# MCG-NKU/E2FGVI

Measured on AMD Instinct MI355X. Metric: inpainted frames/sec at 432x240 T=10, higher is better.
Workload: dtype f32; 1 GPU; BASELINE.json configs[1]: e2fgvi 432x240 T=10 l_t=10, 1 clip(s) per GPU per forward (1 in the job), random-init weights, torch.rand frames + box mask (SURVEY.md 8d); clips_per_gpu=1, precision=fp32, kernel_selection=e2fgvi_amd/tile_table.py (checked in, deterministic: ops.py), hip_graph=True, forwards_in_flight=2

## Files before the change

e2fgvi_amd/build.py:

```python
import os
import subprocess
import sys
from concurrent.futures import ThreadPoolExecutor

HERE = os.path.dirname(os.path.abspath(__file__))
CSRC = os.path.join(HERE, "csrc")
LIB = os.path.join(CSRC, "libe2fgvi_hip.so")
FLAGS = ["--offload-arch=gfx950", "-O3", "-std=c++17", "-fPIC", "-ffp-contract=fast"]
NOPK = ["-Xclang", "-target-feature", "-Xclang", "-packed-fp32-ops"]
UNITS = [("error.hip", "error.o", []), ("conv.hip", "conv.o", []), ("conv.hip", "conv_nopk.o", NOPK + ["-DE2_NOPK_VARIANT"]),
         ("conv_bf16x.hip", "conv_bf16x.o", NOPK), ("conv_wino.hip", "conv_wino.o", NOPK), ("conv_wino.hip", "conv_wino_x3.o", NOPK + ["-DE2_WINO_X3=1"]), ("conv_wino4.hip", "conv_wino4.o", NOPK), ("conv_tail.hip", "conv_tail.o", NOPK),
         ("mdcn.hip", "mdcn.o", NOPK), ("attention.hip", "attention.o", []),
         ("attention_bf16.hip", "attention_bf16.o", NOPK), ("attention_x3.hip", "attention_x3.o", NOPK), ("misc.hip", "misc.o", NOPK),
         ("video.hip", "video.o", NOPK), ("yuv.hip", "yuv.o", NOPK), ("metrics.hip", "metrics.o", NOPK),
         ("mask_track.hip", "mask_track.o", NOPK + ["-ffp-contract=off"]),
         ("defects.hip", "defects.o", NOPK)]
NOPK_OBJECTS = ("conv_nopk.o", "conv_bf16x.o", "conv_wino.o", "conv_wino4.o", "conv_wino_x3.o", "conv_tail.o", "mdcn.o", "attention_bf16.o", "attention_x3.o", "misc.o", "video.o", "yuv.o", "metrics.o", "mask_track.o", "defects.o")
OBJDUMP = "/opt/rocm/lib/llvm/bin/llvm-objdump"


def _hipcc():
    for c in (os.environ.get("HIPCC"), "/opt/rocm/bin/hipcc"):
        if c and os.path.exists(c):
            return c
    return "hipcc"


def _stale(out, deps):
    return (not os.path.exists(out)) or any(os.path.getmtime(d) > os.path.getmtime(out) for d in deps)


def build(force=False, verbose=False, nopk_all=False, lib=None, tag=None, defines=()):
    hipcc = _hipcc()
    if tag:
        nopk_all = False
    objdir = os.path.join(CSRC, ("build_" + tag) if tag else ("build_nopk" if nopk_all else "build"))
    os.makedirs(objdir, exist_ok=True)
    out = lib or (os.path.join(CSRC, "libe2fgvi_hip_%s.so" % tag) if tag else
                  os.path.join(CSRC, "libe2fgvi_hip_nopk.so") if nopk_all else LIB)
    headers = [os.path.join(CSRC, "common.h"), os.path.join(HERE, "..", "include", "e2fgvi_hip.h"), os.path.abspath(__file__)]
    jobs = []
    for src, obj, extra in UNITS:
        sp, op = os.path.join(CSRC, src), os.path.join(objdir, obj)
        if nopk_all and not any(f == "-packed-fp32-ops" for f in extra):
            extra = extra + NOPK
        if force or _stale(op, [sp] + headers):
            jobs.append([hipcc] + FLAGS + extra + list(defines) + ["-c", sp, "-o", op])

    def run(cmd):
        if verbose:
            print(" ".join(cmd), flush=True)
        subprocess.check_call(cmd)

    with ThreadPoolExecutor(max_workers=min(4, max(1, len(jobs)))) as ex:
        list(ex.map(run, jobs))
    objs = [os.path.join(objdir, obj) for _, obj, _ in UNITS]
    if force or jobs or _stale(out, objs):
        run([hipcc, "--offload-arch=gfx950", "-shared", "-fPIC", "-o", out] + objs)
    if jobs:
        verify_isa(objdir)
        if not nopk_all:
            verify_wino_waits(objdir)
            verify_exit_reuse(objdir)
            verify_no_scratch(objdir)
            verify_no_scratch(objdir, "conv_bf16x.o", "conv_halo_x3_kernel", "split-operand halo")
            verify_no_scratch(objdir, "video.o", "restore_u8_kernel", "paste-back")
            verify_no_scratch(objdir, "video.o", "overlay_stats_kernel", "overlay sums")
            verify_no_scratch(objdir, "defects.o", "defect_", "dust and dirt")
            verify_overlay_prefetch(objdir)
            verify_no_pk_u8(objdir)
            verify_no_fma64(objdir)
    return out


def build_variant(tag, *defines):
    return build(tag=tag, defines=defines)


def device_isa(obj):
    import shutil
    import tempfile
    d = tempfile.mkdtemp(prefix="e2isa")
    try:
        local = os.path.join(d, os.path.basename(obj))
        shutil.copy(obj, local)
        subprocess.run([OBJDUMP, "--offloading", os.path.basename(obj)], cwd=d, check=True, stdout=subprocess.DEVNULL,
                       stderr=subprocess.DEVNULL)
        dev = [f for f in os.listdir(d) if "gfx950" in f]
        if not dev:
            return ""
        return subprocess.run([OBJDUMP, "-d", os.path.join(d, dev[0])], check=True, capture_output=True, text=True).stdout
    finally:
        shutil.rmtree(d, ignore_errors=True)


def verify_isa(objdir=None):
    import re
    objdir = objdir or os.path.join(CSRC, "build")
    if not os.path.exists(OBJDUMP):
        return
    for obj in NOPK_OBJECTS:
        isa = device_isa(os.path.join(objdir, obj))
        bad = re.findall(r"v_pk_(?:mul|add|fma)_f32", isa)
        if bad or not isa:
            raise RuntimeError("%s: %s" % (obj, "%d packed-fp32 instructions in a unit that must have none" % len(bad) if isa
                                           else "no gfx950 code object found"))


def verify_no_fma64(objdir=None, obj="mask_track.o"):
    import re
    objdir = objdir or os.path.join(CSRC, "build")
    if not os.path.exists(OBJDUMP):
        return 0
    isa = device_isa(os.path.join(objdir, obj))
    fused = re.findall(r"v_fma(?:c|ak|mk)?_f64", isa)
    if fused or not isa:
        raise RuntimeError("%s: %s" % (obj, "%d fused fp64 multiply-adds in a unit that must round every operation" % len(fused) if isa
                                       else "no gfx950 code object found"))
# ... 324 lines not shown
```

e2fgvi_amd/csrc/conv_bf16x.hip:

```cpp
#include "common.h"

namespace {

typedef __bf16 bf16x8 __attribute__((ext_vector_type(8)));
typedef unsigned int u32x4 __attribute__((ext_vector_type(4)));
typedef __attribute__((address_space(3))) void lds_void;

struct ConvXParams {
    const void* src[E2FGVI_MAX_SRC];
    int ld[E2FGVI_MAX_SRC];
    int coff[E2FGVI_MAX_SRC];
    int cpg[E2FGVI_MAX_SRC];
    unsigned src_bytes[E2FGVI_MAX_SRC];
    int nsrc;
    int N, H, W, Ho, Wo, KH, KW, stride, pad;
    int padx;
    int osy, osx, opy, opx, oH, oW;
    int res_bcast;
    int Cout, Cout_g, Npad;
    int M;
    int tilesM, tilesN;
    int nsteps;
    unsigned wgroup_bytes;
    long long wgroup_elems;
// ... 823 lines not shown
                    for (int tm = 0; tm < TM; ++tm) acc[tm][tn] = __builtin_amdgcn_mfma_f32_32x32x16_bf16(al[tm], bh, acc[tm][tn], 0, 0, 0);
#pragma unroll
                    for (int tm = 0; tm < TM; ++tm) acc[tm][tn] = __builtin_amdgcn_mfma_f32_32x32x16_bf16(ah[tm], bl, acc[tm][tn], 0, 0, 0);
#pragma unroll
                    for (int tm = 0; tm < TM; ++tm) acc[tm][tn] = __builtin_amdgcn_mfma_f32_32x32x16_bf16(am[tm], bm, acc[tm][tn], 0, 0, 0);
#pragma unroll
                    for (int tm = 0; tm < TM; ++tm) acc[tm][tn] = __builtin_amdgcn_mfma_f32_32x32x16_bf16(am[tm], bh, acc[tm][tn], 0, 0, 0);
#pragma unroll
                    for (int tm = 0; tm < TM; ++tm) acc[tm][tn] = __builtin_amdgcn_mfma_f32_32x32x16_bf16(ah[tm], bm, acc[tm][tn], 0, 0, 0);
#pragma unroll
                    for (int tm = 0; tm < TM; ++tm) acc[tm][tn] = __builtin_amdgcn_mfma_f32_32x32x16_bf16(ah[tm], bh, acc[tm][tn], 0, 0, 0);
                }
                __builtin_amdgcn_sched_barrier(0);
#pragma unroll
                for (int pl = 0; pl < 3; ++pl) {
#pragma unroll
                    for (int tn = 0; tn < TN; ++tn) { bq[tn][pl] = bn[tn][pl]; bn[tn][pl] = bn2[tn][pl]; }
#pragma unroll
                    for (int tm = 0; tm < TM; ++tm) aq[tm][pl] = an[tm][pl];
                }
            }
        }
        if (blk + 1 < nblk) {
            __syncthreads();
            store_patch();
            __syncthreads();
        }
    }

    const float* res = reinterpret_cast<const float*>(p.res);
    float* dst = reinterpret_cast<float*>(p.dst);
#pragma unroll
    for (int tn = 0; tn < TN; ++tn) {
        const int co = wn * 32 + i;
        if (co >= p.Cout_g) continue;
        const float bv = p.bias ? p.bias[co] : 0.f;
#pragma unroll
        for (int tm = 0; tm < TM; ++tm) {
#pragma unroll
            for (int r = 0; r < 16; ++r) {
                const int row = (r & 3) + 8 * (r >> 2) + 4 * h;
                const int oy = y0 + 2 * (wm * TM + tm) + (row >> 4), ox = x0 + (row & 15);
                if (oy >= p.Ho || ox >= p.Wo) continue;
                const long long m = ((long long)img * p.Ho + oy) * p.Wo + ox;
                float v = acc[tm][tn][r] + bv;
                if (res) v += res[m * p.res_ld + p.res_coff + co];
                v = apply_act(v, p.act, p.slope);
                dst[m * p.dst_ld + p.dst_coff + co] = v;
            }
        }
    }
}

struct PackX {
    int Cout, groups, KH, KW, nsrc;
    int cpg[E2FGVI_MAX_SRC];
    int Cout_g, Npad, Cin_g, steps_per_tap;
    int kc, ch;
    int tp_cq;
    long long total, wgroup_elems;
};

bool geometry_x(int Cout, int groups, int KH, int KW, int nsrc, const int32_t* cpg, PackX* q, bool f32 = false) {
    q->kc = f32 ? 32 : 64;
    q->ch = f32 ? 4 : 8;
    q->tp_cq = 0;
    if (Cout <= 0 || groups <= 0 || Cout % groups || KH <= 0 || KW <= 0 || nsrc < 1 || nsrc > E2FGVI_MAX_SRC) return false;
    q->Cout = Cout; q->groups = groups; q->KH = KH; q->KW = KW; q->nsrc = nsrc;
    q->Cout_g = Cout / groups;
    q->Npad = round_up(q->Cout_g, 32);
    q->Cin_g = 0;
    q->steps_per_tap = 0;
    for (int s = 0; s < E2FGVI_MAX_SRC; ++s) q->cpg[s] = 0;
    for (int s = 0; s < nsrc; ++s) {
        if (cpg[s] <= 0 || cpg[s] % q->ch) return false;
        q->cpg[s] = cpg[s];
        q->Cin_g += cpg[s];
        q->steps_per_tap += cdiv(cpg[s], q->kc);
    }
    q->wgroup_elems = (long long)KH * KW * q->steps_per_tap * q->kc * q->Npad;
    q->total = q->wgroup_elems * groups;
    return true;
}

__device__ __forceinline__ float pack_value(const float* __restrict__ w, const PackX& p, int g, int step, int koct, int n, int e) {
    if (p.tp_cq) {
        const int L = 8 * step + koct;
        const int tapk = L / p.tp_cq;
        const int chk = (L - tapk * p.tp_cq) * p.ch + e;
        if (tapk < p.KH * p.KW && chk < p.cpg[0] && n < p.Cout_g)
            return w[((long long)n * p.Cin_g + chk) * (p.KH * p.KW) + tapk];
        return 0.f;
    }
    const int tap = step / p.steps_per_tap;
    int blk = step - tap * p.steps_per_tap;
    int s = 0, prefix = 0;
    while (blk >= (p.cpg[s] + p.kc - 1) / p.kc) { blk -= (p.cpg[s] + p.kc - 1) / p.kc; prefix += p.cpg[s]; ++s; }
    const int c = blk * p.kc + koct * p.ch + e;
    if (c < p.cpg[s] && n < p.Cout_g)
        return w[((long long)(g * p.Cout_g + n) * p.Cin_g + prefix + c) * (p.KH * p.KW) + tap];
    return 0.f;
}

template <typename T>
__global__ void pack_conv_weight_x_kernel(const float* __restrict__ w, T* __restrict__ wp, const PackX p) {
    const long long idx = (long long)blockIdx.x * blockDim.x + threadIdx.x;
// ... 37 lines not shown
int launch_x(ConvXParams& p, int groups, hipStream_t st, int mode = 0) {
    p.tilesM = cdiv(p.M, BM);
    p.tilesN = cdiv(p.Cout_g, BN);
    if constexpr (PP) {
        if (mode != 2 || p.tp_cq) {
            e2fgvi_set_error("conv2d_x: the ping-pong tiles (107, 108) are for the split-operand mode without tap-packed weights");
            return E2FGVI_EUNSUP;
        }
        hipLaunchKernelGGL((conv_bf16x_kernel<BM, BN, WGM, WGN, false, 2, true>), dim3(p.tilesM * p.tilesN, groups, 1), dim3(64 * WGM * WGN), 0, st, p);
        E2_LAUNCH_CHECK("conv2d_x");
        return 0;
    } else {
    if (S3 && !(p.KH == 3 && p.KW == 3 && p.stride == 1 && p.pad == 1)) {
        e2fgvi_set_error("conv2d_x: the row-shift tiles (11..17) are for 3x3 stride-1 pad-1 layers");
        return E2FGVI_EINVAL;
    }
    if (mode == 1 || mode == 2) {
        if constexpr (!S3) {
            if (mode == 2)
                hipLaunchKernelGGL((conv_bf16x_kernel<BM, BN, WGM, WGN, false, 2>), dim3(p.tilesM * p.tilesN, groups, 1), dim3(64 * WGM * WGN), 0, st, p);
            else
                hipLaunchKernelGGL((conv_bf16x_kernel<BM, BN, WGM, WGN, false, 1>), dim3(p.tilesM * p.tilesN, groups, 1), dim3(64 * WGM * WGN), 0, st, p);
        } else {
            e2fgvi_set_error("conv2d_x: the row-shift tiles (11..18) take bf16 operands only");
            return E2FGVI_EUNSUP;
        }
    } else if (mode == 3) {
        hipLaunchKernelGGL((conv_bf16x_kernel<BM, BN, WGM, WGN, S3, 3>), dim3(p.tilesM * p.tilesN, groups, 1), dim3(64 * WGM * WGN), 0, st, p);
    } else {
        hipLaunchKernelGGL((conv_bf16x_kernel<BM, BN, WGM, WGN, S3, 0>), dim3(p.tilesM * p.tilesN, groups, 1), dim3(64 * WGM * WGN), 0, st, p);
    }
    E2_LAUNCH_CHECK("conv2d_x");
    return 0;
    }
}

template <int TH, int WGM>
int launch_halo_x3(ConvXParams& p, const e2fgvi_convx_desc* d, hipStream_t st, int mode) {
    const bool ok = mode == 2 && !d->tap_packed && d->KH == 7 && d->KW == 7 && d->stride == 1 && d->pad == 3 && d->groups == 1 &&
                    d->nsrc == 1 && d->src_cpg[0] % 16 == 0 && d->Cout <= 64 && !d->out_grid && !d->res_bcast && !d->dst_nchw &&
                    !d->dst2 && d->dst_dtype == E2FGVI_F32 && (!d->residual || d->res_dtype == E2FGVI_F32) &&
                    d->act != E2FGVI_ACT_DCNPOST;
    if (!ok) {
        e2fgvi_set_error("conv2d_x: the halo tiles (51, 52) take split-operand 7x7 stride-1 pad-3 layers: one fp32 source of a multiple "
                         "of 16 channels, no groups, at most 64 output channels, plain packing, fp32 NHWC result and residual");
        return E2FGVI_EUNSUP;
    }
    p.tilesM = p.N * cdiv(p.Ho, TH) * cdiv(p.Wo, 16);
    p.tilesN = 1;
    if (p.Cout_g <= 32)
        hipLaunchKernelGGL((conv_halo_x3_kernel<7, TH, 32, WGM>), dim3(p.tilesM, 1, 1), dim3(64 * WGM), 0, st, p);
    else
        hipLaunchKernelGGL((conv_halo_x3_kernel<7, TH, 64, WGM>), dim3(p.tilesM, 1, 1), dim3(128 * WGM), 0, st, p);
    E2_LAUNCH_CHECK("conv2d_x");
    return 0;
}

}

static bool geometry_taps(int Cout, int KH, int KW, int cin, PackX* q, bool f32 = false) {
    const int32_t cpg[1] = {cin};
    if (cin > 56 || KW < 2 || !geometry_x(Cout, 1, KH, KW, 1, cpg, q, f32)) return false;
    q->tp_cq = cin / q->ch;
    const int steps = cdiv(KH * KW * q->tp_cq, 8);
    q->wgroup_elems = (long long)steps * q->kc * q->Npad;
    q->total = q->wgroup_elems;
    return true;
}

static int mode_x(const char* who, int32_t code) {
    switch (code) {
        case E2FGVI_BF16: return 0;
        case E2FGVI_F32: return 1;
        case E2FGVI_BF16X3: return 2;
        case E2FGVI_F16: return 3;
        default: break;
    }
    e2fgvi_set_error("%s: mode %d is none of E2FGVI_F32 (0), E2FGVI_BF16 (1), E2FGVI_BF16X3 (2), E2FGVI_F16 (3)", who, code);
    return -1;
}

static bool pack_geometry(const char* who, int mode, int tap_packed, int Cout, int groups, int KH, int KW, int nsrc,
                          const int32_t* src_cpg, PackX* q) {
    const bool f32 = mode == 1 || mode == 2;
    const int ch = f32 ? 4 : 8;
    if (!src_cpg) {
        e2fgvi_set_error("%s: null src_cpg", who);
        return false;
    }
    if (tap_packed) {
        if (groups == 1 && nsrc == 1 && geometry_taps(Cout, KH, KW, src_cpg[0], q, f32)) return true;
        e2fgvi_set_error("%s: tap-packed weights: one source of %d ... 56 channels (multiple of %d), no groups, KW >= 2", who, ch, ch);
        return false;
    }
    if (geometry_x(Cout, groups, KH, KW, nsrc, src_cpg, q, f32)) return true;
    e2fgvi_set_error("%s: bad geometry (channels per source must be multiples of %d)", who, ch);
    return false;
}

extern "C" int64_t e2fgvi_packed_conv_weight_x_size(int32_t mode, int32_t tap_packed, int32_t Cout, int32_t groups, int32_t KH,
                                                    int32_t KW, int32_t nsrc, const int32_t* src_cpg) {
    PackX q;
    const int m = mode_x("packed_conv_weight_x_size", mode);
    if (m < 0 || !pack_geometry("packed_conv_weight_x_size", m, tap_packed, Cout, groups, KH, KW, nsrc, src_cpg, &q)) return E2FGVI_EINVAL;
    return m == 2 ? 3 * q.total : q.total;
}
// ... 89 lines not shown
    p.padx = d->out_grid ? d->pad_left : d->pad;
    p.osy = d->out_grid ? d->out_sy : 0; p.osx = d->out_sx; p.opy = d->out_py; p.opx = d->out_px; p.oH = d->out_H; p.oW = d->out_W;
    p.res_bcast = d->res_bcast;
    p.Cout = d->Cout; p.Cout_g = q.Cout_g; p.Npad = q.Npad;
    p.M = d->N * d->Ho * d->Wo;
    p.nsteps = d->KH * d->KW * q.steps_per_tap;
    p.tp_cq = 0; p.tp_magic = 0; p.tp_magic_cq = 0;
    if (d->tap_packed) {
        PackX qt;
        E2_REQUIRE(d->nsrc == 1 && d->groups == 1 && geometry_taps(d->Cout, d->KH, d->KW, d->src_cpg[0], &qt, f32), E2FGVI_EINVAL,
                   "conv2d_x: tap-packed weights are for one source of <= 56 channels, no groups, KW >= 2");
        E2_REQUIRE(d->tile < 10 || d->tile > 20, E2FGVI_EUNSUP, "conv2d_x: the row-shift tiles do not take tap-packed weights");
        q.wgroup_elems = qt.wgroup_elems;
        p.tp_cq = qt.tp_cq;
        p.tp_magic = 0xFFFFFFFFu / (unsigned)d->KW + 1u;
        p.tp_magic_cq = qt.tp_cq > 1 ? 0xFFFFFFFFu / (unsigned)qt.tp_cq + 1u : 0u;
        p.nsteps = cdiv(d->KH * d->KW * qt.tp_cq, 8);
    }
    p.wgroup_elems = q.wgroup_elems; p.wgroup_bytes = (unsigned)(q.wgroup_elems * wbytes_num);
    p.w = d->wpacked; p.bias = d->bias;
    p.res = d->residual; p.res_ld = d->res_ld; p.res_coff = d->res_coff; p.res_bf16 = d->res_dtype == dt16;
    p.dst = d->dst; p.dst_ld = d->dst_ld; p.dst_coff = d->dst_coff; p.dst_bf16 = d->dst_dtype == dt16;
    p.dst_nchw = d->dst_nchw;
    p.dst2 = (__bf16*)d->dst2; p.dst2_ld = d->dst2_ld; p.dst2_coff = d->dst2_coff;
    p.split_from = d->dst2_split_from; p.split_plane = d->dst2_plane_stride;
    p.act = d->act; p.slope = d->slope;
    hipStream_t st = (hipStream_t)stream;
    int tile = d->tile;
    p.dbg_noload = 0;
    if (tile == 21 || tile == 24 || tile == 26 || tile == 27) { p.dbg_noload = 1; tile -= 20; }
    if (tile == 31 || tile == 34 || tile == 36) { p.dbg_noload = 2; tile -= 30; }
    if (tile == 41 || tile == 44 || tile == 46) { p.dbg_noload = 3; tile -= 40; }
    if (tile == 61 || tile == 66) { p.dbg_noload = 8; tile -= 60; }
    if (tile == 71 || tile == 74 || tile == 76 || tile == 77) { p.dbg_noload = 16; tile -= 70; }
    if (tile == 81 || tile == 84 || tile == 86 || tile == 87) { p.dbg_noload = 32; tile -= 80; }
    if (!tile) {
        if (p.Cout_g <= 32) tile = 3;
        else if (p.Cout_g <= 64) tile = 2;
        else tile = ((long long)cdiv(p.M, 128) * cdiv(p.Cout_g, 128) * d->groups >= 384) ? 1 : 4;
    }
    switch (tile) {
        case 1: return launch_x<128, 128, 2, 2, false>(p, d->groups, st, mode);
        case 2: return launch_x<128, 64, 2, 2, false>(p, d->groups, st, mode);
        case 3: return launch_x<128, 32, 4, 1, false>(p, d->groups, st, mode);
        case 4: return launch_x<64, 128, 2, 2, false>(p, d->groups, st, mode);
        case 5: return launch_x<64, 64, 2, 2, false>(p, d->groups, st, mode);
        case 6: return launch_x<256, 128, 4, 2, false>(p, d->groups, st, mode);
        case 7: return launch_x<256, 256, 4, 2, false>(p, d->groups, st, mode);
        case 8: return launch_x<256, 192, 4, 2, false>(p, d->groups, st, mode);
        case 107: return launch_x<256, 256, 4, 2, false, true>(p, d->groups, st, mode);
        case 108: return launch_x<256, 192, 4, 2, false, true>(p, d->groups, st, mode);
        case 51: return launch_halo_x3<16, 4>(p, d, st, mode);
        case 52: return launch_halo_x3<8, 2>(p, d, st, mode);
        case 11: return launch_x<128, 128, 2, 2, true>(p, d->groups, st, mode);
        case 12: return launch_x<128, 64, 2, 2, true>(p, d->groups, st, mode);
        case 13: return launch_x<128, 32, 4, 1, true>(p, d->groups, st, mode);
        case 14: return launch_x<64, 128, 2, 2, true>(p, d->groups, st, mode);
        case 16: return launch_x<256, 128, 4, 2, true>(p, d->groups, st, mode);
        case 17: return launch_x<256, 256, 4, 2, true>(p, d->groups, st, mode);
        case 18: return launch_x<256, 64, 4, 2, true>(p, d->groups, st, mode);
        default: break;
    }
    e2fgvi_set_error("conv2d_x: unknown tile %d", tile);
    return E2FGVI_EINVAL;
}

extern "C" int e2fgvi_conv2d_x(const e2fgvi_convx_desc* d, int32_t mode, void* stream) {
    const int m = mode_x("conv2d_x", mode);
    return m < 0 ? E2FGVI_EINVAL : conv2d_x(d, stream, m);
}
```

e2fgvi_amd/ops.py:

```python
import collections
import ctypes as C
import math
import numbers
import os

import torch

from . import lib as _L

ACT_NONE, ACT_RELU, ACT_LRELU, ACT_TANH, ACT_DCNPOST = _L.ACT_NONE, _L.ACT_RELU, _L.ACT_LRELU, _L.ACT_TANH, _L.ACT_DCNPOST


def _stream():
    return C.c_void_p(torch.cuda.current_stream().cuda_stream)


def _chk(t, name, dtype=torch.float32):
    if not isinstance(t, torch.Tensor) or not t.is_cuda:
        raise TypeError("%s must be a CUDA (ROCm) tensor -- the HIP path has no CPU fallback" % name)
    if t.dtype != dtype:
        raise TypeError("%s must be %s, got %s" % (name, dtype, t.dtype))
    if not t.is_contiguous():
        raise ValueError("%s must be contiguous" % name)
    return t


def _ptr(t):
    return C.c_void_p(t.data_ptr()) if t is not None else C.c_void_p(0)


def empty_nhwc(n, h, w, c, device):
    return torch.empty((n, h, w, c), dtype=torch.float32, device=device)


TUNE_CANDIDATES = (0, 213, 223, 211, 219, 216)
WINO_CANDIDATES = (64, 132, 164, 32)
W4_CODES = {2464: (2, 64)}
_W4_MINPIX = 20000
XTUNE_CANDIDATES = (1, 4, 6, 7, 8, 2, 5, 3, 107, 108, 51, 52)
XTUNE_HALO = (51, 52)
XTUNE_ROWSHIFT = (11, 16, 17, 12, 13, 18)
X3_ENABLED = os.environ.get("E2FGVI_X3", "1") != "0"
X3_MARGIN = 0.97
X3_BASE = 30000
W3_BASE = 40000
W3_CANDIDATES = (132, 164, 32, 5132, 6064)
W3_WIDE = 6064
W3_WIDE_FALLBACK = 164
DMA_BASE = 2000


def _decode(code):
    if code >= W3_BASE:
        return "w3", code - W3_BASE
    if code >= X3_BASE:
        return "x3", code - X3_BASE
    if code in W4_CODES:
        return "w4", code
    if DMA_BASE <= code < DMA_BASE + 100:
        return "dma", code - DMA_BASE
    return "own", code


_TUNED = {}
AUTOTUNE = os.environ.get("E2FGVI_AUTOTUNE", "0") == "1"
TUNE_REPS = max(1, int(os.environ.get("E2FGVI_TUNE_REPS", "1") or 1))
TABLE_FORMAT = 2
_SIZE_FIELD = 8


def _default_tune_file():
    try:
        st = os.stat(_L.LIB_PATH)
        d = os.environ.get("E2FGVI_CACHE_DIR") or os.path.join(os.path.dirname(os.path.abspath(__file__)), ".tile_cache")
        os.makedirs(d, exist_ok=True)
        dev = "gpu"
        if torch.cuda.is_available():
            dev = "".join(ch for ch in torch.cuda.get_device_properties(0).gcnArchName.split(":")[0] if ch.isalnum())
        return os.path.join(d, "tiles_v%d_%s_%x_%x.txt" % (TABLE_FORMAT, dev, st.st_size, int(st.st_mtime)))
    except (OSError, RuntimeError):
        return None


_TUNE_FILE = None
if AUTOTUNE:
    _TUNE_FILE = os.environ.get("E2FGVI_TUNE_FILE")
    if _TUNE_FILE is None:
        _TUNE_FILE = _default_tune_file()
    elif _TUNE_FILE in ("", "0"):
        _TUNE_FILE = None
    if _TUNE_FILE and os.path.exists(_TUNE_FILE):
        import ast
        for _line in open(_TUNE_FILE):
# ... 600 lines not shown
                     out2=None if out2 is None else out2[n0:n1], tile=tile, **kw)
            return out
        kw.update(out=out, residual=residual, out2=out2)
        d = self._desc(srcs, **kw)
        if planes is not None:
            self._set_planes(d, planes, split_from, N * Ho * Wo)
        if tile == 0 and self.tune and N * Ho * Wo >= 2048:
            family, tile = self._select(d, srcs, kw)
            if family == "x3":
                try:
                    return self.alt3(srcs, out_dtype=out_dtype, tile=tile, planes=planes, split_from=split_from, **kw)
                except _L.HipError:
                    tile = 0
        d.tile = tile
        if _L.TRACE is not None:
            _L.annotate(**self._work(d))
        d.wpacked = self.wpacked.data_ptr()
        rc = self._fn(C.byref(d), _stream())
        if rc != 0 and d.tile and self.tune:
            d.tile = 0
            rc = self._fn(C.byref(d), _stream())
        _L.check(rc, "conv2d_x")
        return out

    def _select(self, d, srcs, kw):
        out, residual = kw["out"], kw["residual"]
        x3 = self.try_x3 and X3_ENABLED and self.f32 and not self.x3
        key = (("x3" if self.x3 else ("x32+3" if x3 else "x32")) if self.f32 else "x", self.Cout, tuple(self.cpg), self.KH, self.KW, self.stride, self.pad, self.groups,
               int(4.0 * math.log2(d.N * d.Ho * d.Wo)), _dt_key(out), kw["out_nchw"], self.taps)
        best = _decision(key)
        if best is None and AUTOTUNE and not torch.cuda.is_current_stream_capturing() and (
                residual is None or residual.data_ptr() != out.data_ptr()):
            best = _remember(key, self._tune(d, srcs, kw, x3))
        if _decode(best or 0)[0] in ("x3", "w3"):
            return ("x3", best - X3_BASE) if self._alt3() is not None else ("own", 0)
        return "own", best or 0

    def _tune(self, d, srcs, kw, x3):
        res = self._time_tiles(d)
        best = min(res, key=res.get) if res else 0
        if x3 and self._alt3() is not None:
            res3 = self.alt3._time_tiles(self.alt3._desc(srcs, **kw))
            if res3 and (not res or min(res3.values()) < X3_MARGIN * min(res.values())):
                best = X3_BASE + min(res3, key=res3.get)
        return best

    def _work(self, d):
        N, H, W, Ho, Wo, tile = d.N, d.H, d.W, d.Ho, d.Wo, d.tile
        cin_g, cout_g, K2 = sum(self.cpg), self.Cout // self.groups, self.KH * self.KW
        kc = 32 if self.f32 else 64
        cin_p = sum(-(-c // kc) * kc for c in self.cpg)
        if self.taps:
            cin_p = -(-K2 * (self.cpg[0] // (4 if self.f32 else 8)) // 8) * kc / K2
        return dict(layer=self.name, kernel="conv_%s tile=%d%s" % (("f32x3" if self.x3 else "f32x") if self.f32 else
                                                                   "f16x" if self.f16 else "bf16x", tile, " taps" if self.taps else ""),
                    shape="N%d %dx%d %d->%d k%d s%d g%d" % (N, H, W, cin_g * self.groups, self.Cout, self.KH, self.stride, self.groups),
                    macs=N * Ho * Wo * self.Cout * cin_g * K2, tile=int(tile),
                    issued=int(N * Ho * Wo * (-(-cout_g // 32) * 32) * self.groups * cin_p * K2 * (_L.X3_PIPE if self.x3 else 1)))

    def _halo_x3(self):
        return (self.x3 and not self.taps and (self.KH, self.KW, self.stride, self.pad, self.groups) == (7, 7, 1, 3, 1)
                and len(self.cpg) == 1 and self.cpg[0] % 16 == 0 and self.Cout <= 64)

    def _time_tiles(self, d, reps=3, rounds=2):
        st = _stream()
        res = {}
        d.tile = 0
        d.wpacked = self.wpacked.data_ptr()

        def run():
            return self._fn(C.byref(d), st)
        for _ in range(2):
            run()
        for _ in range(rounds * TUNE_REPS):
            rowshift = (self.KH, self.KW, self.stride, self.pad) == (3, 3, 1, 1) and not self.f32 and not self.taps
            for code in XTUNE_CANDIDATES + (XTUNE_ROWSHIFT if rowshift else ()):
                if code in XTUNE_HALO and not self._halo_x3():
                    continue
                if code % 10 == 3 and self.Cout // self.groups > 64:
                    continue
                if code in (12, 18) and self.Cout // self.groups > 64:
                    continue
                d.tile = code
                if run() == 0:
                    res[code] = min(res.get(code, float("inf")), _time_launches(run, reps))
        d.tile = 0
        return res


class SoftCompGather:

    def __init__(self, weight, bias, channels=128, dtype=torch.bfloat16):
        w = _chk(weight.detach().float().contiguous(), "weight")
        if w.dim() != 2 or w.shape[0] != 49 * channels:
            raise ValueError("SoftComp embedding weight must be [%d, hidden]" % (49 * channels))
        self.C, self.hidden, self.dtype = channels, w.shape[1], dtype
        w4 = w.view(channels, 7, 7, self.hidden)
        self.phases = []
        for py in range(3):
            ky_taps = [6, 3, 0] if py == 0 else [py + 3, py]
            for px in range(3):
                kx_taps = [6, 3, 0] if px == 0 else [px + 3, px]
                wp = w4[:, ky_taps][:, :, kx_taps].permute(0, 3, 1, 2).contiguous()
                layer = PackedConvX(wp, None, [self.hidden], dtype=dtype)
                layer.name = "sc.embedding phase (%d,%d)" % (py, px)
                self.phases.append((py, px, 1 if py == 0 else 0, 1 if px == 0 else 0, layer))
        self.bias = None if bias is None else _chk(bias.detach().float().contiguous(), "bias")
        self._bias_img = {}
        self.tile = 0

    def bias_image(self, fh, fw):
        if self.bias is None:
            return None

        def build():
            rows = self.bias.view(self.C, 49).t().reshape(1, 49 * self.C).expand(fh * fw, 49 * self.C).contiguous()
            return softcomp_fold(rows, 1, fh, fw, 3 * fh, 3 * fw, self.C)[0].contiguous()
        return _lazy(self._bias_img, (fh, fw), "sc.embedding (folded bias image)", build)

    def __call__(self, tokens, out=None, out_dtype=None):
        _chk(tokens, "tokens", self.dtype)
        F_, fh, fw, hid = tokens.shape
        if hid != self.hidden:
            raise ValueError("tokens must be [F, fh, fw, %d]" % self.hidden)
        H, W = 3 * fh, 3 * fw
        if out is None:
            out = torch.empty((F_, H, W, self.C), dtype=out_dtype or self.dtype, device=tokens.device)
        if tuple(out.shape) != (F_, H, W, self.C):
            raise ValueError("out must be [%d,%d,%d,%d]" % (F_, H, W, self.C))
        chunks = list(_image_chunks(F_, fh * fw * hid * tokens.element_size()))
# ... 1036 lines not shown
```

e2fgvi_amd/tile_table.py:

```python
TABLE_FORMAT = 2
TILES = {
    ('x', 128, (128, 128), 1, 1, 1, 0, 1, 63, 1, False, False): 1,
    ('x', 128, (128, 128), 1, 1, 1, 0, 1, 76, 1, False, False): 4,
    ('x', 128, (128, 128), 1, 1, 1, 0, 1, 85, 1, False, False): 4,
    ('x', 128, (128, 128), 3, 3, 1, 1, 1, 50, 1, False, False): 5,
    ('x', 128, (128, 128), 3, 3, 1, 1, 1, 63, 1, False, False): 1,
    ('x', 128, (128, 128), 3, 3, 1, 1, 1, 68, 1, False, False): 4,
    ('x', 128, (128, 128, 128), 3, 3, 1, 1, 1, 50, 1, False, False): 5,
    ('x', 128, (128, 128, 128), 3, 3, 1, 1, 1, 63, 1, False, False): 11,
    ('x', 128, (128, 128, 128), 3, 3, 1, 1, 1, 68, 1, False, False): 4,
    ('x', 128, (128, 128, 128, 8), 3, 3, 1, 1, 1, 50, 1, False, False): 5,
    ('x', 128, (128, 128, 128, 8), 3, 3, 1, 1, 1, 63, 1, False, False): 11,
    ('x', 128, (128, 128, 128, 8), 3, 3, 1, 1, 1, 68, 1, False, False): 11,
    ('x', 128, (128,), 3, 3, 1, 1, 1, 50, 1, False, False): 5,
    ('x', 128, (128,), 3, 3, 1, 1, 1, 63, 1, False, False): 6,
    ('x', 128, (128,), 3, 3, 1, 1, 1, 68, 1, False, False): 4,
    ('x', 128, (128,), 3, 3, 1, 1, 1, 71, 1, False, False): 1,
    ('x', 128, (128,), 3, 3, 1, 1, 1, 76, 1, False, False): 1,
    ('x', 128, (128,), 3, 3, 1, 1, 1, 84, 1, False, False): 1,
    ('x', 128, (128,), 3, 3, 1, 1, 1, 85, 1, False, False): 6,
    ('x', 128, (128,), 3, 3, 1, 1, 1, 93, 1, False, False): 6,
    ('x', 128, (256, 256), 3, 3, 1, 1, 1, 63, 1, False, False): 16,
    ('x', 128, (256, 256), 3, 3, 1, 1, 1, 76, 1, False, False): 11,
    ('x', 128, (256, 256), 3, 3, 1, 1, 1, 85, 1, False, False): 11,
# ... 255 lines not shown
    (32, (64,), 7, 7, 1, 3, 1, 32, 49, False, 1, False, False, 0, 'x3'): 0,
    (32, (64,), 7, 7, 1, 3, 1, 32, 52, False, 1, False, False, 0, 'x3'): 0,
    (32, (64,), 7, 7, 1, 3, 1, 32, 53, False, 1, False, False, 0, 'x3'): 0,
    (32, (64,), 7, 7, 1, 3, 1, 32, 56, False, 1, False, False, 0, 'x3'): 0,
    (32, (64,), 7, 7, 1, 3, 1, 32, 57, False, 1, False, False, 0, 'x3'): 0,
    (32, (64,), 7, 7, 1, 3, 1, 32, 60, False, 1, False, False, 0, 'x3'): 30051,
    (32, (64,), 7, 7, 1, 3, 1, 32, 61, False, 1, False, False, 0, 'x3'): 30003,
    (32, (64,), 7, 7, 1, 3, 1, 32, 64, False, 1, False, False, 0, 'x3'): 30003,
    (32, (64,), 7, 7, 1, 3, 1, 32, 65, False, 1, False, False, 0, 'x3'): 30003,
    (32, (64,), 7, 7, 1, 3, 1, 32, 68, False, 1, False, False, 0, 'x3'): 30051,
    (32, (64,), 7, 7, 1, 3, 1, 32, 69, False, 1, False, False, 0, 'x3'): 30003,
    (32, (64,), 7, 7, 1, 3, 1, 32, 72, False, 1, False, False, 0, 'x3'): 30003,
    (32, (64,), 7, 7, 1, 3, 1, 32, 73, False, 1, False, False, 0, 'x3'): 30003,
    (32, (64,), 7, 7, 1, 3, 1, 32, 80, False, 1, False, False, 0, 'x3'): 30003,
    (32, (8,), 7, 7, 1, 3, 1, 8, 44, False, 1, False, False, 0, 'x3'): 0,
    (32, (8,), 7, 7, 1, 3, 1, 8, 45, False, 1, False, False, 0, 'x3'): 0,
    (32, (8,), 7, 7, 1, 3, 1, 8, 48, False, 1, False, False, 0, 'x3'): 0,
    (32, (8,), 7, 7, 1, 3, 1, 8, 49, False, 1, False, False, 0, 'x3'): 0,
    (32, (8,), 7, 7, 1, 3, 1, 8, 52, False, 1, False, False, 0, 'x3'): 0,
    (32, (8,), 7, 7, 1, 3, 1, 8, 53, False, 1, False, False, 0, 'x3'): 0,
    (32, (8,), 7, 7, 1, 3, 1, 8, 56, False, 1, False, False, 0, 'x3'): 0,
    (32, (8,), 7, 7, 1, 3, 1, 8, 57, False, 1, False, False, 0, 'x3'): 0,
    (32, (8,), 7, 7, 1, 3, 1, 8, 60, False, 1, False, False, 0, 'x3'): 0,
    (32, (8,), 7, 7, 1, 3, 1, 8, 61, False, 1, False, False, 0, 'x3'): 0,
    (32, (8,), 7, 7, 1, 3, 1, 8, 64, False, 1, False, False, 0, 'x3'): 0,
    (32, (8,), 7, 7, 1, 3, 1, 8, 65, False, 1, False, False, 0, 'x3'): 0,
    (32, (8,), 7, 7, 1, 3, 1, 8, 68, False, 1, False, False, 0, 'x3'): 0,
    (32, (8,), 7, 7, 1, 3, 1, 8, 69, False, 1, False, False, 0, 'x3'): 0,
    (32, (8,), 7, 7, 1, 3, 1, 8, 72, False, 1, False, False, 0, 'x3'): 0,
    (32, (8,), 7, 7, 1, 3, 1, 8, 73, False, 1, False, False, 0, 'x3'): 0,
    (32, (8,), 7, 7, 1, 3, 1, 8, 80, False, 1, False, False, 0, 'x3'): 0,
    (384, (256,), 3, 3, 1, 1, 1, 32, 59, False, 2, True, False, 2464, 'x3'): 46064,
    (384, (256,), 3, 3, 1, 1, 1, 32, 63, False, 2, True, False, 2464, 'x3'): 46064,
    (384, (256,), 3, 3, 1, 1, 1, 32, 67, False, 2, True, False, 2464, 'x3'): 46064,
    (384, (256,), 3, 3, 1, 1, 1, 32, 68, False, 2, True, False, 0, 'x3'): 46064,
    (384, (256,), 3, 3, 1, 1, 1, 32, 75, False, 2, True, False, 2464, 'x3'): 46064,
    (384, (64, 128), 3, 3, 1, 1, 4, 32, 59, False, 2, True, False, 0, 'x3'): 45132,
    (384, (64, 128), 3, 3, 1, 1, 4, 32, 63, False, 2, True, False, 0, 'x3'): 45132,
    (384, (64, 128), 3, 3, 1, 1, 4, 32, 67, False, 2, True, False, 0, 'x3'): 45132,
    (384, (64, 128), 3, 3, 1, 1, 4, 32, 68, False, 2, True, False, 0, 'x3'): 46064,
    (384, (64, 128), 3, 3, 1, 1, 4, 32, 75, False, 2, True, False, 0, 'x3'): 46064,
    (432, (128,), 3, 3, 1, 1, 1, 32, 50, True, 4, True, False, 0, 'x3'): 46064,
    (432, (128,), 3, 3, 1, 1, 1, 32, 54, True, 4, True, False, 0, 'x3'): 46064,
    (432, (128,), 3, 3, 1, 1, 1, 32, 55, True, 4, True, False, 0, 'x3'): 46064,
    (432, (128,), 3, 3, 1, 1, 1, 32, 62, True, 4, True, False, 0, 'x3'): 46064,
    (512, (128, 192), 3, 3, 1, 1, 2, 32, 59, False, 2, True, False, 2464, 'x3'): 46064,
    (512, (128, 192), 3, 3, 1, 1, 2, 32, 63, False, 2, True, False, 2464, 'x3'): 46064,
    (512, (128, 192), 3, 3, 1, 1, 2, 32, 67, False, 2, True, False, 2464, 'x3'): 46064,
    (512, (128, 192), 3, 3, 1, 1, 2, 32, 68, False, 2, True, False, 0, 'x3'): 46064,
    (512, (128, 192), 3, 3, 1, 1, 2, 32, 75, False, 2, True, False, 2464, 'x3'): 46064,
    (512, (128,), 7, 7, 3, 3, 1, 32, 47, False, 0, False, True, 0): 2005,
    (512, (128,), 7, 7, 3, 3, 1, 32, 47, False, 0, False, True, 0, 'x3'): 30005,
    (512, (128,), 7, 7, 3, 3, 1, 32, 51, False, 0, False, True, 0): 2004,
    (512, (128,), 7, 7, 3, 3, 1, 32, 51, False, 0, False, True, 0, 'x3'): 30004,
    (512, (128,), 7, 7, 3, 3, 1, 32, 54, False, 0, False, True, 0): 2005,
    (512, (128,), 7, 7, 3, 3, 1, 32, 54, False, 0, False, True, 0, 'x3'): 30006,
    (512, (128,), 7, 7, 3, 3, 1, 32, 55, False, 0, False, True, 0): 2001,
    (512, (128,), 7, 7, 3, 3, 1, 32, 55, False, 0, False, True, 0, 'x3'): 30001,
    (512, (128,), 7, 7, 3, 3, 1, 32, 63, False, 0, False, True, 0): 2004,
    (512, (128,), 7, 7, 3, 3, 1, 32, 63, False, 0, False, True, 0, 'x3'): 30107,
    (512, (1960,), 1, 1, 1, 0, 1, 32, 47, True, 0, False, True, 0): 2005,
    (512, (1960,), 1, 1, 1, 0, 1, 32, 51, True, 0, False, True, 0): 2004,
    (512, (1960,), 1, 1, 1, 0, 1, 32, 54, True, 0, False, True, 0): 2005,
    (512, (1960,), 1, 1, 1, 0, 1, 32, 55, True, 0, False, True, 0): 2001,
    (512, (1960,), 1, 1, 1, 0, 1, 32, 63, True, 0, False, True, 0): 2004,
    (512, (512,), 1, 1, 1, 0, 1, 32, 47, True, 0, False, True, 0): 2005,
    (512, (512,), 1, 1, 1, 0, 1, 32, 47, True, 0, False, True, 0, 'x3'): 30005,
    (512, (512,), 1, 1, 1, 0, 1, 32, 51, True, 0, False, True, 0): 2004,
    (512, (512,), 1, 1, 1, 0, 1, 32, 51, True, 0, False, True, 0, 'x3'): 30004,
    (512, (512,), 1, 1, 1, 0, 1, 32, 54, True, 0, False, True, 0): 2005,
    (512, (512,), 1, 1, 1, 0, 1, 32, 54, True, 0, False, True, 0, 'x3'): 30001,
    (512, (512,), 1, 1, 1, 0, 1, 32, 55, True, 0, False, True, 0): 2001,
    (512, (512,), 1, 1, 1, 0, 1, 32, 55, True, 0, False, True, 0, 'x3'): 30001,
    (512, (512,), 1, 1, 1, 0, 1, 32, 63, True, 0, False, True, 0): 2005,
    (512, (512,), 1, 1, 1, 0, 1, 32, 63, True, 0, False, True, 0, 'x3'): 30107,
    (6272, (512,), 1, 1, 1, 0, 1, 32, 47, False, 0, False, True, 0): 2004,
    (6272, (512,), 1, 1, 1, 0, 1, 32, 47, False, 0, False, True, 0, 'x3'): 30108,
    (6272, (512,), 1, 1, 1, 0, 1, 32, 51, False, 0, False, True, 0): 2004,
    (6272, (512,), 1, 1, 1, 0, 1, 32, 51, False, 0, False, True, 0, 'x3'): 30107,
    (6272, (512,), 1, 1, 1, 0, 1, 32, 54, False, 0, False, True, 0): 2007,
    (6272, (512,), 1, 1, 1, 0, 1, 32, 54, False, 0, False, True, 0, 'x3'): 30107,
    (6272, (512,), 1, 1, 1, 0, 1, 32, 55, False, 0, False, True, 0): 2002,
    (6272, (512,), 1, 1, 1, 0, 1, 32, 55, False, 0, False, True, 0, 'x3'): 30107,
    (6272, (512,), 1, 1, 1, 0, 1, 32, 63, False, 0, False, True, 0): 2007,
    (6272, (512,), 1, 1, 1, 0, 1, 32, 63, False, 0, False, True, 0, 'x3'): 30107,
    (64, (128,), 3, 3, 1, 1, 1, 32, 67, False, 2, True, False, 0, 'x3'): 46064,
    (64, (128,), 3, 3, 1, 1, 1, 32, 71, False, 2, True, False, 0, 'x3'): 46064,
    (64, (128,), 3, 3, 1, 1, 1, 32, 75, False, 2, True, False, 0, 'x3'): 46064,
    (64, (128,), 3, 3, 1, 1, 1, 32, 76, False, 2, True, False, 0, 'x3'): 46064,
    (64, (128,), 3, 3, 1, 1, 1, 32, 83, False, 2, True, False, 0, 'x3'): 46064,
    (64, (32,), 7, 7, 1, 3, 1, 32, 44, False, 1, False, False, 0, 'x3'): 0,
    (64, (32,), 7, 7, 1, 3, 1, 32, 45, False, 1, False, False, 0, 'x3'): 0,
    (64, (32,), 7, 7, 1, 3, 1, 32, 48, False, 1, False, False, 0, 'x3'): 0,
    (64, (32,), 7, 7, 1, 3, 1, 32, 49, False, 1, False, False, 0, 'x3'): 0,
    (64, (32,), 7, 7, 1, 3, 1, 32, 52, False, 1, False, False, 0, 'x3'): 30052,
    (64, (32,), 7, 7, 1, 3, 1, 32, 53, False, 1, False, False, 0, 'x3'): 0,
    (64, (32,), 7, 7, 1, 3, 1, 32, 56, False, 1, False, False, 0, 'x3'): 0,
    (64, (32,), 7, 7, 1, 3, 1, 32, 57, False, 1, False, False, 0, 'x3'): 30005,
    (64, (32,), 7, 7, 1, 3, 1, 32, 60, False, 1, False, False, 0, 'x3'): 30051,
    (64, (32,), 7, 7, 1, 3, 1, 32, 61, False, 1, False, False, 0, 'x3'): 30005,
    (64, (32,), 7, 7, 1, 3, 1, 32, 64, False, 1, False, False, 0, 'x3'): 30002,
    (64, (32,), 7, 7, 1, 3, 1, 32, 65, False, 1, False, False, 0, 'x3'): 30005,
    (64, (32,), 7, 7, 1, 3, 1, 32, 68, False, 1, False, False, 0, 'x3'): 30052,
    (64, (32,), 7, 7, 1, 3, 1, 32, 69, False, 1, False, False, 0, 'x3'): 30005,
    (64, (32,), 7, 7, 1, 3, 1, 32, 72, False, 1, False, False, 0, 'x3'): 30005,
    (64, (32,), 7, 7, 1, 3, 1, 32, 73, False, 1, False, False, 0, 'x3'): 30005,
    (64, (32,), 7, 7, 1, 3, 1, 32, 80, False, 1, False, False, 0, 'x3'): 30005,
# ... 15 lines not shown
```

Measured before the change: 964.2 frames/s.

## Add halo-tiled split-bf16 kernel for 7x7 stride-3 convolution

Adds a dedicated split-operand (3x bf16) MFMA kernel for 7x7 stride-3 pad-3 convolutions. Each workgroup stages an input halo patch in LDS, de-interleaved by column phase, and reuses it across all 49 taps while weights stream through a register pipeline. This targets the redundant global/im2col traffic of the generic path. The tile table switches one 512-channel stride-3 layer at 51 rows to the new tile, and the autotuner and cost model learn the new codes. Output tiles of 5x6 use 30 of 32 MFMA rows, wasting some compute.

```diff
diff --git a/e2fgvi_amd/build.py b/e2fgvi_amd/build.py
--- a/e2fgvi_amd/build.py
+++ b/e2fgvi_amd/build.py
@@ -64,6 +64,7 @@
             verify_exit_reuse(objdir)
             verify_no_scratch(objdir)
             verify_no_scratch(objdir, "conv_bf16x.o", "conv_halo_x3_kernel", "split-operand halo")
+            verify_no_scratch(objdir, "conv_bf16x.o", "conv_halo_s3_x3_kernel", "split-operand stride-3 halo")
             verify_no_scratch(objdir, "video.o", "restore_u8_kernel", "paste-back")
             verify_no_scratch(objdir, "video.o", "overlay_stats_kernel", "overlay sums")
             verify_no_scratch(objdir, "defects.o", "defect_", "dust and dirt")
diff --git a/e2fgvi_amd/csrc/conv_bf16x.hip b/e2fgvi_amd/csrc/conv_bf16x.hip
--- a/e2fgvi_amd/csrc/conv_bf16x.hip
+++ b/e2fgvi_amd/csrc/conv_bf16x.hip
@@ -899,6 +899,216 @@
     }
 }
 
+template <int TMY, int TMX, int BN, int TN>
+__global__ __launch_bounds__(64 * (BN / (32 * TN))) __attribute__((amdgpu_waves_per_eu(2))) void conv_halo_s3_x3_kernel(const ConvXParams p) {
+    constexpr int TM = TMY * TMX;
+    constexpr int TH = 5 * TMY, TW = 6 * TMX;
+    constexpr int PH = 3 * (TH - 1) + 7, PW = 3 * (TW - 1) + 7, NPIX = PH * PW;
+    constexpr int PWC = TW + 2;
+    constexpr int RP = (3 * PWC + 13) / 16 * 16 + 2;
+    constexpr int PLANE = PH * RP * 16;
+    constexpr int WGN = BN / (32 * TN);
+    constexpr int NT = 64 * WGN;
+    constexpr int P_IT = (NPIX + NT - 1) / NT;
+    constexpr int NJ = 25;
+    constexpr int BD = 2;
+    constexpr unsigned OOB = 0xFFFFFFFFu;
+    constexpr int NP = TM / 2;
+    static_assert(RP >= 3 * PWC && RP % 16 == 2 && 3 * PLANE <= 160 * 1024 && 2 * PLANE + 7 * RP * 16 < 65536, "patch");
+    static_assert(TM == 2 * NP && (NP == 1 || NP == 2), "sub-tile pairs");
+
+    __shared__ __attribute__((aligned(16))) unsigned char smem[3 * PLANE];
+
+    const int tid = threadIdx.x;
+    const int lane = tid & 63, wn = tid >> 6;
+    const int tiles_x = (p.Wo + TW - 1) / TW, tiles_y = (p.Ho + TH - 1) / TH;
+    int sp = xcd_remap(blockIdx.x, p.tilesM * p.tilesN);
+    const int n0 = (sp / p.tilesM) * BN;
+    sp %= p.tilesM;
+    const int txi = sp % tiles_x;
+    sp /= tiles_x;
+    const int tyi = sp % tiles_y;
+    const int img = sp / tiles_y;
+    const int y0 = tyi * TH, x0 = txi * TW;
+
+    int pp_pix[P_IT], pp_lds[P_IT];
+#pragma unroll
+    for (int it = 0; it < P_IT; ++it) {
+        const int f = tid + it * NT;
+        const int py = f / PW, px = f - py * PW;
+        const int iy = 3 * y0 - 3 + py, ix = 3 * x0 - 3 + px;
+        const bool ok = f < NPIX && iy >= 0 && iy < p.H && ix >= 0 && ix < p.W;
+        pp_pix[it] = ok ? (img * p.H + iy) * p.W + ix : -1;
+        pp_lds[it] = (py * RP + (px % 3) * PWC + px / 3) * 16;
+    }
+    const __amdgpu_buffer_rsrc_t arsrc = make_rsrc(p.src[0], p.src_bytes[0]);
+    const unsigned ld4 = (unsigned)p.ld[0] * 4u;
+    const unsigned chan = (unsigned)p.coff[0] * 4u;
+    const int nblk = p.cpg[0] >> 3;
+
+    f32x4 rp[P_IT][2];
+    auto load_patch = [&](int blk) {
+#pragma unroll
+        for (int it = 0; it < P_IT; ++it) {
+            const bool ok = blk < nblk && pp_pix[it] >= 0;
+            const unsigned off = (unsigned)pp_pix[it] * ld4 + chan + (unsigned)blk * 32u;
+            rp[it][0] = __builtin_bit_cast(f32x4, __builtin_amdgcn_raw_buffer_load_b128(arsrc, (int)(ok ? off : OOB), 0, 0));
+            rp[it][1] = __builtin_bit_cast(f32x4, __builtin_amdgcn_raw_buffer_load_b128(arsrc, (int)(ok ? off + 16u : OOB), 0, 0));
+        }
+    };
+    auto store_patch = [&]() {
+#pragma unroll
+        for (int it = 0; it < P_IT; ++it) {
+            if (NPIX % NT == 0 || (tid + it * NT) < NPIX) {
+                bf16x8 sh, sm, sl;
+                split8(rp[it][0], rp[it][1], sh, sm, sl);
+                *reinterpret_cast<bf16x8*>(smem + pp_lds[it]) = sh;
+                *reinterpret_cast<bf16x8*>(smem + PLANE + pp_lds[it]) = sm;
+                *reinterpret_cast<bf16x8*>(smem + 2 * PLANE + pp_lds[it]) = sl;
+            }
+        }
+    };
+
+    const int i = lane & 31;
+    const int h = lane >> 5;
+    int hm = -h;
+    const int lty = i < 30 ? i / 6 : 0, ltx = i < 30 ? i - lty * 6 : i - 16;
+    int a_base[TM];
+#pragma unroll
+    for (int tm = 0; tm < TM; ++tm) a_base[tm] = (3 * (5 * (tm / TMX) + lty) * RP + 6 * (tm % TMX) + ltx) * 16;
+    auto load_a = [&](bf16x8 (&a)[2][3], int pr, int j) {
+        const int t0 = 2 * j, t1 = 2 * j + 1 < 49 ? 2 * j + 1 : 48;
+        const int o0 = ((t0 / 7) * RP + ((t0 % 7) % 3) * PWC + (t0 % 7) / 3) * 16;
+        const int o1 = ((t1 / 7) * RP + ((t1 % 7) % 3) * PWC + (t1 % 7) / 3) * 16;
+        const int o = hm & (o1 - o0);
+#pragma unroll
+        for (int tm = 0; tm < 2; ++tm)
+#pragma unroll
+            for (int pl = 0; pl < 3; ++pl) a[tm][pl] = *reinterpret_cast<const bf16x8*>(smem + pl * PLANE + o0 + a_base[2 * pr + tm] + o);
+    };
+
+    const __amdgpu_buffer_rsrc_t wrsrc = make_rsrc(p.w, p.wgroup_bytes);
+    unsigned b_col[TN];
+#pragma unroll
+    for (int tn = 0; tn < TN; ++tn) {
+        const int col = n0 + (wn * TN + tn) * 32 + i;
+        b_col[tn] = col < p.Npad ? (unsigned)col * 16u : OOB;
+    }
+    const unsigned oct_bytes = (unsigned)p.Npad * 16u;
+    const unsigned plane_bytes = 4u * oct_bytes, step_bytes = 3u * plane_bytes;
+    const int opt = p.tp_cq ? p.tp_cq >> 1 : ((p.cpg[0] + 31) >> 5) * 4;
+    auto load_b = [&](bf16x8 (&b)[TN][3], int j, int blk) {
+        const int oc0 = 2 * j * opt + blk, oc1 = oc0 + opt;
+        const unsigned s0 = (unsigned)(oc0 >> 2) * step_bytes + (unsigned)(oc0 & 3) * oct_bytes;
+        const unsigned s1 = (unsigned)(oc1 >> 2) * step_bytes + (unsigned)(oc1 & 3) * oct_bytes;
+        const bool live0 = blk < nblk, live1 = live0 && 2 * j + 1 < 49;
+        const unsigned so = h ? s1 : s0;
+        const bool live = h ? live1 : live0;
+#pragma unroll
+        for (int tn = 0; tn < TN; ++tn) {
+            const unsigned voff = (live && b_col[tn] != OOB) ? b_col[tn] + so : OOB;
+#pragma unroll
+            for (int pl = 0; pl < 3; ++pl)
+                b[tn][pl] = __builtin_bit_cast(bf16x8, __builtin_amdgcn_raw_buffer_load_b128(wrsrc, (int)voff, (int)((unsigned)pl * plane_bytes), 0));
+        }
+    };
+
+    f32x16 acc[TM][TN];
+#pragma unroll
+    for (int tm = 0; tm < TM; ++tm)
+#pragma unroll
+        for (int tn = 0; tn < TN; ++tn)
+#pragma unroll
+            for (int r = 0; r < 16; ++r) acc[tm][tn][r] = 0.f;
+
+    bf16x8 bs[BD + 1][TN][3], aq[NP][2][3], an[2][3];
+    load_patch(0);
+#pragma unroll
+    for (int k = 0; k < BD; ++k) load_b(bs[k], k, 0);
+    store_patch();
+    __syncthreads();
+
+    auto mma_pair = [&](const bf16x8 (&a)[2][3], int pr) {
+#pragma unroll
+        for (int tn = 0; tn < TN; ++tn) {
+            const bf16x8 bh = bs[0][tn][0], bm = bs[0][tn][1], bl = bs[0][tn][2];
+#pragma unroll
+            for (int tm = 0; tm < 2; ++tm) acc[2 * pr + tm][tn] = __builtin_amdgcn_mfma_f32_32x32x16_bf16(a[tm][2], bh, acc[2 * pr + tm][tn], 0, 0, 0);
+#pragma unroll
+            for (int tm = 0; tm < 2; ++tm) acc[2 * pr + tm][tn] = __builtin_amdgcn_mfma_f32_32x32x16_bf16(a[tm][0], bl, acc[2 * pr + tm][tn], 0, 0, 0);
+#pragma unroll
+            for (int tm = 0; tm < 2; ++tm) acc[2 * pr + tm][tn] = __builtin_amdgcn_mfma_f32_32x32x16_bf16(a[tm][1], bm, acc[2 * pr + tm][tn], 0, 0, 0);
+#pragma unroll
+            for (int tm = 0; tm < 2; ++tm) acc[2 * pr + tm][tn] = __builtin_amdgcn_mfma_f32_32x32x16_bf16(a[tm][1], bh, acc[2 * pr + tm][tn], 0, 0, 0);
+#pragma unroll
+            for (int tm = 0; tm < 2; ++tm) acc[2 * pr + tm][tn] = __builtin_amdgcn_mfma_f32_32x32x16_bf16(a[tm][0], bm, acc[2 * pr + tm][tn], 0, 0, 0);
+#pragma unroll
+            for (int tm = 0; tm < 2; ++tm) acc[2 * pr + tm][tn] = __builtin_amdgcn_mfma_f32_32x32x16_bf16(a[tm][0], bh, acc[2 * pr + tm][tn], 0, 0, 0);
+        }
+    };
+
+    for (int blk = 0; blk < nblk; ++blk) {
+        asm volatile("" : "+v"(hm));
+        load_patch(blk + 1);
+        load_a(aq[0], 0, 0);
+#pragma unroll
+        for (int j = 0; j < NJ; ++j) {
+            load_b(bs[BD], j + BD < NJ ? j + BD : j + BD - NJ, j + BD < NJ ? blk : blk + 1);
+            if (NP == 2) load_a(aq[NP - 1], 1, j);
+            else if (j + 1 < NJ) load_a(an, 0, j + 1);
+            __builtin_amdgcn_sched_barrier(0);
+            mma_pair(aq[0], 0);
+            __builtin_amdgcn_sched_barrier(0);
+            if (NP == 2) {
+                if (j + 1 < NJ) load_a(an, 0, j + 1);
+                __builtin_amdgcn_sched_barrier(0);
+                mma_pair(aq[NP - 1], 1);
+                __builtin_amdgcn_sched_barrier(0);
+            }
+#pragma unroll
+            for (int pl = 0; pl < 3; ++pl) {
+#pragma unroll
+                for (int tn = 0; tn < TN; ++tn)
+#pragma unroll
+                    for (int k = 0; k < BD; ++k) bs[k][tn][pl] = bs[k + 1][tn][pl];
+                if (j + 1 < NJ) {
+#pragma unroll
+                    for (int tm = 0; tm < 2; ++tm) aq[0][tm][pl] = an[tm][pl];
+                }
+            }
+        }
+        if (blk + 1 < nblk) {
+            __syncthreads();
+            store_patch();
+            __syncthreads();
+        }
+    }
+
+    const float* res = reinterpret_cast<const float*>(p.res);
+    float* dst = reinterpret_cast<float*>(p.dst);
+#pragma unroll
+    for (int tn = 0; tn < TN; ++tn) {
+        const int co = n0 + (wn * TN + tn) * 32 + i;
+        if (co >= p.Cout_g) continue;
+        const float bv = p.bias ? p.bias[co] : 0.f;
+#pragma unroll
+        for (int tm = 0; tm < TM; ++tm) {
+#pragma unroll
+            for (int r = 0; r < 16; ++r) {
+                const int row = (r & 3) + 8 * (r >> 2) + 4 * h;
+                const int ty = row / 6;
+                const int oy = y0 + 5 * (tm / TMX) + ty, ox = x0 + 6 * (tm % TMX) + row - 6 * ty;
+                if (row >= 30 || oy >= p.Ho || ox >= p.Wo) continue;
+                const long long m = ((long long)img * p.Ho + oy) * p.Wo + ox;
+                float v = acc[tm][tn][r] + bv;
+                if (res) v += res[m * p.res_ld + p.res_coff + co];
+                v = apply_act(v, p.act, p.slope);
+                dst[m * p.dst_ld + p.dst_coff + co] = v;
+            }
+        }
+    }
+}
+
 struct PackX {
     int Cout, groups, KH, KW, nsrc;
     int cpg[E2FGVI_MAX_SRC];
@@ -1042,6 +1252,23 @@
         hipLaunchKernelGGL((conv_halo_x3_kernel<7, TH, 32, WGM>), dim3(p.tilesM, 1, 1), dim3(64 * WGM), 0, st, p);
     else
         hipLaunchKernelGGL((conv_halo_x3_kernel<7, TH, 64, WGM>), dim3(p.tilesM, 1, 1), dim3(128 * WGM), 0, st, p);
+    E2_LAUNCH_CHECK("conv2d_x");
+    return 0;
+}
+
+template <int TMY, int BN, int TN>
+int launch_halo_s3_x3(ConvXParams& p, const e2fgvi_convx_desc* d, hipStream_t st, int mode) {
+    const bool ok = mode == 2 && d->KH == 7 && d->KW == 7 && d->stride == 3 && d->pad == 3 && d->groups == 1 && d->nsrc == 1 &&
+                    d->src_cpg[0] % 8 == 0 && !d->out_grid && !d->res_bcast && !d->dst_nchw && !d->dst2 &&
+                    d->dst_dtype == E2FGVI_F32 && (!d->residual || d->res_dtype == E2FGVI_F32) && d->act != E2FGVI_ACT_DCNPOST;
+    if (!ok) {
+        e2fgvi_set_error("conv2d_x: the stride-3 halo tiles (54, 56) take split-operand 7x7 stride-3 pad-3 layers: one fp32 source of a "
+                         "multiple of 8 channels, no groups, fp32 NHWC result and residual, no second output");
+        return E2FGVI_EUNSUP;
+    }
+    p.tilesM = p.N * cdiv(p.Ho, 5 * TMY) * cdiv(p.Wo, 12);
+    p.tilesN = cdiv(p.Cout_g, BN);
+    hipLaunchKernelGGL((conv_halo_s3_x3_kernel<TMY, 2, BN, TN>), dim3(p.tilesM * p.tilesN, 1, 1), dim3(64 * (BN / (32 * TN))), 0, st, p);
     E2_LAUNCH_CHECK("conv2d_x");
     return 0;
 }
@@ -1237,6 +1464,8 @@
         case 108: return launch_x<256, 192, 4, 2, false, true>(p, d->groups, st, mode);
         case 51: return launch_halo_x3<16, 4>(p, d, st, mode);
         case 52: return launch_halo_x3<8, 2>(p, d, st, mode);
+        case 54: return launch_halo_s3_x3<2, 128, 1>(p, d, st, mode);
+        case 56: return launch_halo_s3_x3<1, 128, 1>(p, d, st, mode);
         case 11: return launch_x<128, 128, 2, 2, true>(p, d->groups, st, mode);
         case 12: return launch_x<128, 64, 2, 2, true>(p, d->groups, st, mode);
         case 13: return launch_x<128, 32, 4, 1, true>(p, d->groups, st, mode);
diff --git a/e2fgvi_amd/ops.py b/e2fgvi_amd/ops.py
--- a/e2fgvi_amd/ops.py
+++ b/e2fgvi_amd/ops.py
@@ -37,8 +37,9 @@
 WINO_CANDIDATES = (64, 132, 164, 32)
 W4_CODES = {2464: (2, 64)}
 _W4_MINPIX = 20000
-XTUNE_CANDIDATES = (1, 4, 6, 7, 8, 2, 5, 3, 107, 108, 51, 52)
+XTUNE_CANDIDATES = (1, 4, 6, 7, 8, 2, 5, 3, 107, 108, 51, 52, 54, 56)
 XTUNE_HALO = (51, 52)
+XTUNE_HALO_S3 = {54: 10, 56: 5}
 XTUNE_ROWSHIFT = (11, 16, 17, 12, 13, 18)
 X3_ENABLED = os.environ.get("E2FGVI_X3", "1") != "0"
 X3_MARGIN = 0.97
@@ -745,15 +746,24 @@
         cin_p = sum(-(-c // kc) * kc for c in self.cpg)
         if self.taps:
             cin_p = -(-K2 * (self.cpg[0] // (4 if self.f32 else 8)) // 8) * kc / K2
+        rows, cols = N * Ho * Wo, -(-cout_g // 32) * 32
+        if tile in XTUNE_HALO_S3 and self._halo_s3_x3():
+            th = XTUNE_HALO_S3[tile]
+            rows, cols = N * -(-Ho // th) * -(-Wo // 12) * (th // 5) * 64, -(-cout_g // 128) * 128
+            cin_p = self.cpg[0] // 8 * 25 * 16 / K2
         return dict(layer=self.name, kernel="conv_%s tile=%d%s" % (("f32x3" if self.x3 else "f32x") if self.f32 else
                                                                    "f16x" if self.f16 else "bf16x", tile, " taps" if self.taps else ""),
                     shape="N%d %dx%d %d->%d k%d s%d g%d" % (N, H, W, cin_g * self.groups, self.Cout, self.KH, self.stride, self.groups),
                     macs=N * Ho * Wo * self.Cout * cin_g * K2, tile=int(tile),
-                    issued=int(N * Ho * Wo * (-(-cout_g // 32) * 32) * self.groups * cin_p * K2 * (_L.X3_PIPE if self.x3 else 1)))
+                    issued=int(rows * cols * self.groups * cin_p * K2 * (_L.X3_PIPE if self.x3 else 1)))
 
     def _halo_x3(self):
         return (self.x3 and not self.taps and (self.KH, self.KW, self.stride, self.pad, self.groups) == (7, 7, 1, 3, 1)
                 and len(self.cpg) == 1 and self.cpg[0] % 16 == 0 and self.Cout <= 64)
+
+    def _halo_s3_x3(self):
+        return (self.x3 and (self.KH, self.KW, self.stride, self.pad, self.groups) == (7, 7, 3, 3, 1)
+                and len(self.cpg) == 1 and self.cpg[0] % 8 == 0)
 
     def _time_tiles(self, d, reps=3, rounds=2):
         st = _stream()
@@ -769,6 +779,8 @@
             rowshift = (self.KH, self.KW, self.stride, self.pad) == (3, 3, 1, 1) and not self.f32 and not self.taps
             for code in XTUNE_CANDIDATES + (XTUNE_ROWSHIFT if rowshift else ()):
                 if code in XTUNE_HALO and not self._halo_x3():
+                    continue
+                if code in XTUNE_HALO_S3 and not self._halo_s3_x3():
                     continue
                 if code % 10 == 3 and self.Cout // self.groups > 64:
                     continue
diff --git a/e2fgvi_amd/tile_table.py b/e2fgvi_amd/tile_table.py
--- a/e2fgvi_amd/tile_table.py
+++ b/e2fgvi_amd/tile_table.py
@@ -331,7 +331,7 @@
     (512, (128,), 7, 7, 3, 3, 1, 32, 47, False, 0, False, True, 0): 2005,
     (512, (128,), 7, 7, 3, 3, 1, 32, 47, False, 0, False, True, 0, 'x3'): 30005,
     (512, (128,), 7, 7, 3, 3, 1, 32, 51, False, 0, False, True, 0): 2004,
-    (512, (128,), 7, 7, 3, 3, 1, 32, 51, False, 0, False, True, 0, 'x3'): 30004,
+    (512, (128,), 7, 7, 3, 3, 1, 32, 51, False, 0, False, True, 0, 'x3'): 30056,
     (512, (128,), 7, 7, 3, 3, 1, 32, 54, False, 0, False, True, 0): 2005,
     (512, (128,), 7, 7, 3, 3, 1, 32, 54, False, 0, False, True, 0, 'x3'): 30006,
     (512, (128,), 7, 7, 3, 3, 1, 32, 55, False, 0, False, True, 0): 2001,
```

New measurement: 944.0 frames/s. 0.979x the previous value.
